# Openflight-sim/OPEN_Ludwig

Hardware: AMD Instinct MI355X
Metric: MLUPS (million lattice updates/s) at 256^3 D3Q27; % of HBM roofline (higher is better)
Workload: dtype f32

## Files before the change

open_ludwig_amd/csrc/kernels.hpp:

```cpp
#pragma once

#include <hip/hip_runtime.h>
#include <stdint.h>
#include <type_traits>

#include "lattice.hpp"
#include "jl_math.h"

namespace lw {

struct SCParams {
    const float *f_in;
    float *f_out;
    float *f_post;
    const uint32_t *post_rows;
    const float *vel_in;
    float *vel_out;
    float *rho;
    const uint8_t *obstacle;
    const float *sponge;
    const float *wall_dist;
    const int32_t *meta;
    const int32_t *items;
    const float *pf_new, *pf_old, *prho_new, *prho_old, *pvel_new, *pvel_old;
// ... 495 lines not shown

    const float tr_gsq = gsq11 + gsq22 + gsq33;
    const float tr_term = tr_gsq / 3.0f;
    const float Sd11 = gsq11 - tr_term, Sd22 = gsq22 - tr_term, Sd33 = gsq33 - tr_term;
    const float Sd12 = 0.5f * (gsq12 + gsq21), Sd13 = 0.5f * (gsq13 + gsq31), Sd23 = 0.5f * (gsq23 + gsq32);
    const float S12 = 0.5f * (g12 + g21), S13 = 0.5f * (g13 + g31), S23 = 0.5f * (g23 + g32);
    const float OP1 = Sd11 * Sd11 + Sd22 * Sd22 + Sd33 * Sd33 + 2.0f * (Sd12 * Sd12 + Sd13 * Sd13 + Sd23 * Sd23);
    const float OP2 = g11 * g11 + g22 * g22 + g33 * g33 + 2.0f * (S12 * S12 + S13 * S13 + S23 * S23);

    float nu_eddy = 0.0f;
    if (OP1 > 1.0e-12f) {
        const float OP1_32 = OP1 * sqrtf(OP1);
        const float OP2_52 = OP2 * OP2 * sqrtf(jl_max(OP2, 1.0e-12f));
        const float denom = OP2_52 + OP1 * sqrtf(sqrtf(jl_max(OP1, 1.0e-12f)));
        if (denom > 1.0e-12f) nu_eddy = (p.c_wale * p.c_wale) * OP1_32 / denom;
    }
    nu_eddy = jl_max(nu_eddy, p.nu_bg);
    const float tau_turb = p.tau + nu_eddy * 3.0f;
    const float omega = 1.0f / jl_max(tau_turb, 0.500001f);

    Chain2<PACKED> P_x, P_y, P_z;
    static_for<0, Q>([&](auto kc) {
        constexpr int k = decltype(kc)::value, ko = OPP(k);
        constexpr int cx = CX(k), cy = CY(k), cz = CZ(k);
        float f_neq;
        if constexpr (PACKED && k < ko) {
            const float cu = cdot<k>(ux_eq, uy_eq, uz_eq);
            const f32x2 both = f32x2{fs[k], fs[ko]} - equilibrium_value<f32x2>(rho, WEIGHT(k), f32x2{cu, -cu}, usq_eq);
            f_neq = both.x;
            fs[ko] = both.y;
        } else if constexpr (PACKED && k > ko) {
            f_neq = fs[k];
        } else {
            f_neq = fs[k] - equilibrium_value<float>(rho, WEIGHT(k), cdot<k>(ux_eq, uy_eq, uz_eq), usq_eq);
        }
        if constexpr (cx * cy != 0) P_x.add_both(f_neq, cx * cy > 0 ? f_neq : -f_neq);
        else if constexpr (cx != 0) P_x.add_first(f_neq);
        if constexpr (cy * cz != 0) P_y.add_both(f_neq, cy * cz > 0 ? f_neq : -f_neq);
        else if constexpr (cy != 0) P_y.add_first(f_neq);
        if constexpr (cz * cx != 0) P_z.add_both(f_neq, cz * cx > 0 ? f_neq : -f_neq);
        else if constexpr (cz != 0) P_z.add_first(f_neq);
    });
    const float Pi_xx = P_x.first(), Pi_xy = P_x.second(), Pi_yy = P_y.first(), Pi_yz = P_y.second(), Pi_zz = P_z.first(), Pi_zx = P_z.second();

    const float one_m_omega = 1.0f - omega;
    const float one_m_half_omega = 1.0f - 0.5f * omega;
    if constexpr (REC_OUT) {
        store_record(p.rec_out, own, rho, ux_eq, uy_eq, uz_eq, Pi_xx, Pi_yy, Pi_zz, Pi_xy, Pi_yz, Pi_zx, one_m_omega);
        return;
    }
    static_for<0, Q>([&](auto kc) {
        constexpr int k = decltype(kc)::value;
        float f_coll = collide_value<k>(rho, ux_eq, uy_eq, uz_eq, Pi_xx, Pi_yy, Pi_zz, Pi_xy, Pi_yz, Pi_zx, one_m_omega);
        if constexpr (WALL) {
            constexpr float w_k = WEIGHT(k);
            constexpr float cx_f = (float)CX(k), cy_f = (float)CY(k), cz_f = (float)CZ(k);
            const float cu = cdot<k>(ux_eq, uy_eq, uz_eq);
            const float force_term = (w_k * 3.0f) * ((cx_f - ux + 3.0f * cu * cx_f) * Fx + (cy_f - uy + 3.0f * cu * cy_f) * Fy +
                                                     (cz_f - uz + 3.0f * cu * cz_f) * Fz);
            f_coll = f_coll + one_m_half_omega * force_term;
        }
        if constexpr (POST) { if (store_post) st_f32(p.f_post, own.b, F_BLOCK_BYTES, k * COMP_BYTES + own.cell4, f_coll); }
        st_f32(p.f_out, own.b, F_BLOCK_BYTES, k * COMP_BYTES + own.cell4, f_coll);
    });
}

__device__ __forceinline__ void finish_rho_only(const SCParams &p, const int flags, const Own own, const float (&fs)[Q])
{
    float rho = 0.0f;
    static_for<0, Q>([&](auto kc) { rho += fs[decltype(kc)::value]; });
    bool is_obs = false;
    if (flags & FLAG_HAS_OBSTACLE) is_obs = p.obstacle[(size_t)own.b * CELLS + (own.cell4 >> 2)] != 0;
    if (is_obs) { st_f32(p.rho, own.b, S_BLOCK_BYTES, own.cell4, 1.0f); return; }
    rho = jl_max(rho, 0.01f);
    if (flags & FLAG_HAS_SPONGE) {
        const float sp = ld_own(p.sponge, own.b, S_BLOCK_BYTES, own.cell4);
        if (sp > 0.0f) rho = rho * (1.0f - sp) + 1.0f * sp;
    }
    st_f32(p.rho, own.b, S_BLOCK_BYTES, own.cell4, rho);
}

__device__ __forceinline__ void patch_missing_sources(const SCParams &p, const int32_t *__restrict__ meta, const NeighbourIds &nbr,
                                                      const LanePos &l, const int z, const Own own, float (&fs)[Q])
{
    const int gx = (meta[NBR_BX] - 1) * BS + l.x + 1, gy = (meta[NBR_BY] - 1) * BS + l.y + 1, gz = (meta[NBR_BZ] - 1) * BS + z + 1;
    const float *iface_own = p.is_level_1 == 0 ? p.f_iface + (size_t)meta[NBR_GBI] * CELLS + (own.cell4 >> 2) : nullptr;
    static_for<0, Q>([&](auto kc) {
        constexpr int k = decltype(kc)::value;
        constexpr int cx = CX(k), cy = CY(k), cz = CZ(k);
        if constexpr (k != 13) {
            if (source_block<k>(nbr, l) < 0) {
                const int src_gx = gx - cx, src_gy = gy - cy, src_gz = gz - cz;
                const bool is_inlet = src_gx < 1, is_outlet = src_gx > p.nx_g;
                const bool is_y_min = src_gy < 1, is_y_max = src_gy > p.ny_g;
                const bool is_z_min = src_gz < 1, is_z_max = src_gz > p.nz_g;
                float val;
                if (is_inlet) {
                    const float noise = p.inlet_turbulence > 0.0f
                                            ? gradient_noise(gy, gz, p.seed, 1234) * p.inlet_turbulence * p.u_inlet
                                            : 0.0f;
                    const float u_inst = p.u_inlet + noise;
                    const float cu_in = (float)cx * u_inst;
                    val = WEIGHT(k) * (1.0f + 3.0f * cu_in + 4.5f * cu_in * cu_in - 1.5f * u_inst * u_inst);
                } else if (is_outlet) {
                    const float cu_out = (float)cx * p.u_inlet;
                    val = WEIGHT(k) * (1.0f + 3.0f * cu_out + 4.5f * cu_out * cu_out - 1.5f * p.u_inlet * p.u_inlet);
                } else if (is_y_min && p.is_symmetric == 1) {
                    val = ld_own(p.f_in, own.b, F_BLOCK_BYTES, MIRROR_Y(k) * COMP_BYTES + own.cell4);
                } else if (is_y_min || is_y_max) {
                    val = ld_own(p.f_in, own.b, F_BLOCK_BYTES, MIRROR_Y(k) * COMP_BYTES + own.cell4);
                } else if (is_z_min || is_z_max) {
                    val = ld_own(p.f_in, own.b, F_BLOCK_BYTES, MIRROR_Z(k) * COMP_BYTES + own.cell4);
                } else if (p.is_level_1 == 0) {
                    val = iface_own[(size_t)k * p.n_iface_blocks * CELLS];
                } else {
                    val = WEIGHT(k);
                }
                fs[k] = val;
            }
        }
    });
}

__device__ __forceinline__ float dpp_from_lower_lane(float v)
{
    return __int_as_float(__builtin_amdgcn_update_dpp(__float_as_int(v), __float_as_int(v), 0x111, 0xF, 0xF, false));
}
__device__ __forceinline__ float dpp_from_upper_lane(float v)
{
    return __int_as_float(__builtin_amdgcn_update_dpp(__float_as_int(v), __float_as_int(v), 0x101, 0xF, 0xF, false));
}
__host__ __device__ constexpr int XSLOT(int k) { return CX(k) == 1 ? k / 3 : 9 + k / 3; }

constexpr int ITEM_LINK_W = 1 << 30;
constexpr int ITEM_LINK_E = 1 << 29;
constexpr int ITEM_ID_MASK = (1 << 29) - 1;

#ifndef LW_MIN_WAVES
#define LW_MIN_WAVES 5
#endif
template <int NW, bool GENERAL, bool POST, bool WALL, bool RHO_ONLY, bool WIDE, bool REC_OUT>
__device__ __forceinline__ void stream_collide_xrun(const SCParams p)
{
    __shared__ float xch[NW][24][8];
    const int wave = __builtin_amdgcn_readfirstlane(threadIdx.x >> 6);
    const int raw = p.items[blockIdx.x * NW + wave];
    const bool active = raw >= 0;
    const int item = active ? (raw & ITEM_ID_MASK) : 0;
    const int b = item >> 3;
    const int z = item & 7;
    const int lane = threadIdx.x & 63;
    LanePos l;
    l.x = lane & 7; l.y = lane >> 3;
    l.x0 = l.x == 0; l.x7 = l.x == 7; l.y0 = l.y == 0; l.y7 = l.y == 7;
    const int32_t *__restrict__ meta = p.meta + (size_t)b * NBR_STRIDE;
    const int flags = meta[NBR_FLAGS];
    const NeighbourIds nbr = load_neighbour_ids(meta, z);
    const Own own{b, (uint32_t)((l.x + 8 * l.y + 64 * z) * 4)};
    const bool first = !active || (raw & ITEM_LINK_W) == 0, last = !active || (raw & ITEM_LINK_E) == 0;
    float fs[Q];
    float halo[Q];
    float uc[3], uT[3], uB[3], uy_edge[3], ux_edge_lo[3], ux_edge_hi[3];
    if (active) {
    static_for<0, Q>([&](auto kc) {
        constexpr int k = decltype(kc)::value;
        constexpr int cx = CX(k), cy = CY(k), g = 1 - CZ(k);
        const bool yo = cy == 1 ? l.y0 : (cy == -1 ? l.y7 : false);
        const int c00 = nbr.id[g][4], cY = nbr.id[g][4 - 3 * cy];
        int sel = cy != 0 ? (yo ? cY : c00) : c00;
        if constexpr (GENERAL) sel = sel >= 0 ? sel : b;
        const uint32_t rowz = (uint32_t)(k * COMP_BYTES) + (uint32_t)((8 * ((l.y - cy) & 7)) * 4) + (uint32_t)(nbr.zs[g] * 256);
        if constexpr (cy == 0) fs[k] = ld_f32<true>(p.f_in, sel, F_BLOCK_BYTES, rowz + (uint32_t)(l.x * 4));
        else fs[k] = ld_f32<WIDE>(p.f_in, sel, F_BLOCK_BYTES, rowz + (uint32_t)(l.x * 4));
        halo[k] = 0.0f;
        if constexpr (cx != 0) {
            if (cx == 1 ? first : last) {
                const int cX = nbr.id[g][4 - cx], cXY = nbr.id[g][4 - cx - 3 * cy];
                int selx = cy != 0 ? (yo ? cXY : cX) : cX;
                if constexpr (GENERAL) selx = selx >= 0 ? selx : b;
                if (cx == 1 ? l.x0 : l.x7)
                    halo[k] = ld_f32<(cy == 0) || WIDE>(p.f_in, selx, F_BLOCK_BYTES, rowz + (uint32_t)((cx == 1 ? 7 : 0) * 4));
            }
        }
    });
    if constexpr (!RHO_ONLY) {
        int bT = z == 7 ? nbr.id[2][4] : b, bB = z == 0 ? nbr.id[0][4] : b;
        const uint32_t xy = (uint32_t)((l.x + 8 * l.y) * 4);
        uint32_t inT = xy + (uint32_t)(((z + 1) & 7) * 256), inB = xy + (uint32_t)(((z - 1) & 7) * 256);
        int by_ = l.y0 ? nbr.id[1][4 - 3] : nbr.id[1][4 + 3];
        uint32_t inY = (uint32_t)((l.x + 8 * (l.y0 ? 7 : 0) + 64 * z) * 4);
        int bXlo = nbr.id[1][4 - 1], bXhi = nbr.id[1][4 + 1];
        uint32_t inXlo = (uint32_t)((7 + 8 * l.y + 64 * z) * 4), inXhi = (uint32_t)((0 + 8 * l.y + 64 * z) * 4);
        if constexpr (GENERAL) {
            if (bT < 0) { bT = b; inT = own.cell4; }
            if (bB < 0) { bB = b; inB = own.cell4; }
            if (by_ < 0) { by_ = b; inY = own.cell4; }
            if (bXlo < 0) { bXlo = b; inXlo = own.cell4; }
            if (bXhi < 0) { bXhi = b; inXhi = own.cell4; }
        }
#pragma unroll
        for (int c = 0; c < 3; ++c) {
            const uint32_t cb = (uint32_t)c * COMP_BYTES;
            uc[c] = ld_own(p.vel_in, b, V_BLOCK_BYTES, cb + own.cell4);
            uT[c] = ld_own(p.vel_in, bT, V_BLOCK_BYTES, cb + inT);
            uB[c] = ld_own(p.vel_in, bB, V_BLOCK_BYTES, cb + inB);
            uy_edge[c] = 0.0f; ux_edge_lo[c] = 0.0f; ux_edge_hi[c] = 0.0f;
            if (l.y0 || l.y7) uy_edge[c] = ld_f32<WIDE>(p.vel_in, by_, V_BLOCK_BYTES, cb + inY);
            if (first) { if (l.x0) ux_edge_lo[c] = ld_own(p.vel_in, bXlo, V_BLOCK_BYTES, cb + inXlo); }
            if (last) { if (l.x7) ux_edge_hi[c] = ld_own(p.vel_in, bXhi, V_BLOCK_BYTES, cb + inXhi); }
        }
    }

    static_for<0, Q>([&](auto kc) {
        constexpr int k = decltype(kc)::value;
        constexpr int cx = CX(k);
        if constexpr (cx == 1) { if (l.x7) xch[wave][XSLOT(k)][l.y] = fs[k]; }
        if constexpr (cx == -1) { if (l.x0) xch[wave][XSLOT(k)][l.y] = fs[k]; }
    });
    if constexpr (!RHO_ONLY) {
#pragma unroll
        for (int c = 0; c < 3; ++c) {
            if (l.x7) xch[wave][18 + c][l.y] = uc[c];
            if (l.x0) xch[wave][21 + c][l.y] = uc[c];
        }
    }
    }
    __syncthreads();
    if (!active) return;
    const int wlo = first ? 0 : wave - 1, whi = last ? NW - 1 : wave + 1;
    static_for<0, Q>([&](auto kc) {
        constexpr int k = decltype(kc)::value;
        constexpr int cx = CX(k);
        if constexpr (cx == 1) {
            const float inner = dpp_from_lower_lane(fs[k]);
            const float edge = first ? halo[k] : xch[wlo][XSLOT(k)][l.y];
            fs[k] = l.x0 ? edge : inner;
        }
        if constexpr (cx == -1) {
            const float inner = dpp_from_upper_lane(fs[k]);
            const float edge = last ? halo[k] : xch[whi][XSLOT(k)][l.y];
            fs[k] = l.x7 ? edge : inner;
        }
    });
    const bool needs_patch = GENERAL && (flags & FLAG_ALL_NEIGHBOURS) == 0;
    if constexpr (RHO_ONLY) {
        if constexpr (GENERAL) { if (needs_patch) patch_missing_sources(p, meta, nbr, l, z, own, fs); }
        finish_rho_only(p, flags, own, fs);
        return;
    }
    float uE[3], uW[3], uN[3], uS[3];
#pragma unroll
    for (int c = 0; c < 3; ++c) {
        const float e_edge = last ? ux_edge_hi[c] : xch[whi][21 + c][l.y];
        const float w_edge = first ? ux_edge_lo[c] : xch[wlo][18 + c][l.y];
        const float e_in = dpp_from_upper_lane(uc[c]), w_in = dpp_from_lower_lane(uc[c]);
        uE[c] = l.x7 ? e_edge : e_in;
        uW[c] = l.x0 ? w_edge : w_in;
        const float n_in = __shfl_down(uc[c], 8, 64), s_in = __shfl_up(uc[c], 8, 64);
        uN[c] = l.y7 ? uy_edge[c] : n_in;
        uS[c] = l.y0 ? uy_edge[c] : s_in;
    }
    if constexpr (GENERAL) { if (needs_patch) patch_missing_sources(p, meta, nbr, l, z, own, fs); }
    finish_cell<POST, WALL, REC_OUT>(p, flags, own, fs, uE[0], uE[1], uE[2], uW[0], uW[1], uW[2], uN[0], uN[1], uN[2], uS[0], uS[1], uS[2],
                                     uT[0], uT[1], uT[2], uB[0], uB[1], uB[2]);
}
template <int NW, bool GENERAL, bool POST, bool WALL, bool RHO_ONLY = false, bool WIDE = false>
__global__ __launch_bounds__(64 * NW) __attribute__((amdgpu_waves_per_eu((WIDE && GENERAL) ? LW_MIN_WAVES - 1 : LW_MIN_WAVES))) void k_stream_collide_xrun(const SCParams p)
{
    stream_collide_xrun<NW, GENERAL, POST, WALL, RHO_ONLY, WIDE, false>(p);
}
template <int NW, bool WIDE>
__global__ __launch_bounds__(64 * NW) __attribute__((amdgpu_waves_per_eu(LW_MIN_WAVES))) void k_records_from_populations(const SCParams p)
{
    stream_collide_xrun<NW, false, false, false, false, WIDE, true>(p);
}

#ifndef LW_REC_WAVES
#define LW_REC_WAVES 4
#endif
#ifndef LW_REC_AHEAD
#define LW_REC_AHEAD 3
#endif
template <int NW, bool WIDE>
__global__ __launch_bounds__(64 * NW) __attribute__((amdgpu_waves_per_eu(LW_REC_WAVES))) void k_step_records(const SCParams p)
{
    __shared__ float xch[NW][24][8];
    const int wave = __builtin_amdgcn_readfirstlane(threadIdx.x >> 6);
    const int raw = p.items[blockIdx.x * NW + wave];
    const bool active = raw >= 0;
    const int item = active ? (raw & ITEM_ID_MASK) : 0;
    const int b = item >> 3;
    const int z = item & 7;
    const int lane = threadIdx.x & 63;
    LanePos l;
    l.x = lane & 7; l.y = lane >> 3;
    l.x0 = l.x == 0; l.x7 = l.x == 7; l.y0 = l.y == 0; l.y7 = l.y == 7;
    const int32_t *__restrict__ meta = p.meta + (size_t)b * NBR_STRIDE;
    const NeighbourIds nbr = load_neighbour_ids(meta, z);
    const Own own{b, (uint32_t)((l.x + 8 * l.y + 64 * z) * 4)};
    const bool first = !active || (raw & ITEM_LINK_W) == 0, last = !active || (raw & ITEM_LINK_E) == 0;
    __shared__ float xedge[NW][2][12][8];
    float fs[Q];
    float uc[3], uT[3], uB[3], uN[3], uS[3];
    if (active) {
    auto face_rows = [&](auto sc) {
        constexpr int side = decltype(sc)::value;
        constexpr int jx = side == 0 ? 4 - 1 : 4 + 1;
        const int j = l.x;
        const int jz = (j >= 3 ? 1 : 0) + (j >= 6 ? 1 : 0);
        const int cy = j - 3 * jz - 1, cz = jz - 1, g = 2 - jz;
        auto by_g = [&](int v0, int v1, int v2) { return g == 0 ? v0 : (g == 1 ? v1 : v2); };
        const int bX = by_g(nbr.id[0][jx], nbr.id[1][jx], nbr.id[2][jx]);
        const int bXlo = by_g(nbr.id[0][jx - 3], nbr.id[1][jx - 3], nbr.id[2][jx - 3]);
        const int bXhi = by_g(nbr.id[0][jx + 3], nbr.id[1][jx + 3], nbr.id[2][jx + 3]);
        const int blk = (cy == 1 && l.y0) ? bXlo : ((cy == -1 && l.y7) ? bXhi : bX);
        const int zsrc = by_g(nbr.zs[0], nbr.zs[1], nbr.zs[2]);
        float r[R_COMP];
        load_record_at(r, p.rec_in, record_offset<WIDE>(blk, zsrc) + (uint32_t)(((side == 0 ? 7 : 0) + 8 * ((l.y - cy) & 7)) * 4));
        float(&mine)[12][8] = xedge[wave][side];
        mine[j][l.y] = record_face(DirLaneFace{cy, cz}, r, side == 0);
        if (j == 4) { mine[9][l.y] = r[R_UX]; mine[10][l.y] = r[R_UY]; mine[11][l.y] = r[R_UZ]; }
    };
    if (first) face_rows(std::integral_constant<int, 0>{});
    if (last) face_rows(std::integral_constant<int, 1>{});
    if ((first && l.x0) || (last && l.x7)) {
        constexpr int j = 8, cy = 1, g = 0;
        const int wX = nbr.id[g][4 - 1], wXY = nbr.id[g][4 - 1 - 3 * cy], eX = nbr.id[g][4 + 1], eXY = nbr.id[g][4 + 1 - 3 * cy];
        const auto oW = record_offset<WIDE>(wX, nbr.zs[g]), oWY = record_offset<WIDE>(wXY, nbr.zs[g]);
        const auto oE = record_offset<WIDE>(eX, nbr.zs[g]), oEY = record_offset<WIDE>(eXY, nbr.zs[g]);
        const auto off = l.x0 ? (l.y0 ? oWY : oW) : (l.y0 ? oEY : oE);
        float r[R_COMP];
        load_record_at(r, p.rec_in, off + (uint32_t)(((l.x0 ? 7 : 0) + 8 * ((l.y - cy) & 7)) * 4));
        xedge[wave][l.x0 ? 0 : 1][j][l.y] = record_face(DirConst<DIR(1, 1, 1)>{}, r, l.x0);
    }
    __builtin_amdgcn_sched_barrier(0);
    {
        float r[9][R_COMP];
        auto load_pulled = [&](auto jc) {
            constexpr int j = decltype(jc)::value;
            constexpr int cy = j % 3 - 1, g = 1 - (j / 3 - 1);
            const uint32_t lane4 = (uint32_t)((l.x + 8 * ((l.y - cy) & 7)) * 4);
            if constexpr (cy == 0) {
                load_record(r[j], record_plane(p.rec_in, nbr.id[g][4], nbr.zs[g]), lane4);
            } else {
                const bool yo = cy == 1 ? l.y0 : l.y7;
                const auto o0 = record_offset<WIDE>(nbr.id[g][4], nbr.zs[g]), oY = record_offset<WIDE>(nbr.id[g][4 - 3 * cy], nbr.zs[g]);
                load_record_at(r[j], p.rec_in, (yo ? oY : o0) + lane4);
            }
        };
        static_for<0, LW_REC_AHEAD>(load_pulled);
        static_for<0, 9>([&](auto jc) {
            constexpr int j = decltype(jc)::value;
            constexpr int cy = j % 3 - 1, cz = j / 3 - 1;
            if constexpr (j + LW_REC_AHEAD < 9) load_pulled(std::integral_constant<int, j + LW_REC_AHEAD>{});
            __builtin_amdgcn_sched_barrier(0);
            const float(&q)[R_COMP] = r[j];
            record_row<cy, cz>(fs, q);
            if constexpr (cy == 0 && cz == 0) { uc[0] = q[R_UX]; uc[1] = q[R_UY]; uc[2] = q[R_UZ]; }
            if constexpr (cy == 0 && cz == 1) { uB[0] = q[R_UX]; uB[1] = q[R_UY]; uB[2] = q[R_UZ]; }
            if constexpr (cy == 0 && cz == -1) { uT[0] = q[R_UX]; uT[1] = q[R_UY]; uT[2] = q[R_UZ]; }
            if constexpr (cy == 1 && cz == 0) { uS[0] = q[R_UX]; uS[1] = q[R_UY]; uS[2] = q[R_UZ]; }
            if constexpr (cy == -1 && cz == 0) { uN[0] = q[R_UX]; uN[1] = q[R_UY]; uN[2] = q[R_UZ]; }
            __builtin_amdgcn_sched_barrier(0);
        });
    }
    static_for<0, Q>([&](auto kc) {
        constexpr int k = decltype(kc)::value;
        constexpr int cx = CX(k);
        if constexpr (cx == 1) { if (l.x7) xch[wave][XSLOT(k)][l.y] = fs[k]; }
        if constexpr (cx == -1) { if (l.x0) xch[wave][XSLOT(k)][l.y] = fs[k]; }
    });
#pragma unroll
    for (int c = 0; c < 3; ++c) {
        if (l.x7) xch[wave][18 + c][l.y] = uc[c];
        if (l.x0) xch[wave][21 + c][l.y] = uc[c];
    }
    }
    __syncthreads();
    if (!active) return;
    const int wlo = first ? 0 : wave - 1, whi = last ? NW - 1 : wave + 1;
    static_for<0, Q>([&](auto kc) {
        constexpr int k = decltype(kc)::value;
        constexpr int cx = CX(k);
        if constexpr (cx == 1) {
            const float inner = dpp_from_lower_lane(fs[k]);
            const float edge = first ? xedge[wave][0][k / 3][l.y] : xch[wlo][XSLOT(k)][l.y];
            fs[k] = l.x0 ? edge : inner;
        }
        if constexpr (cx == -1) {
            const float inner = dpp_from_upper_lane(fs[k]);
            const float edge = last ? xedge[wave][1][k / 3][l.y] : xch[whi][XSLOT(k)][l.y];
            fs[k] = l.x7 ? edge : inner;
        }
    });
    float uE[3], uW[3];
#pragma unroll
    for (int c = 0; c < 3; ++c) {
        const float e_edge = last ? xedge[wave][1][9 + c][l.y] : xch[whi][21 + c][l.y];
        const float w_edge = first ? xedge[wave][0][9 + c][l.y] : xch[wlo][18 + c][l.y];
        const float e_in = dpp_from_upper_lane(uc[c]), w_in = dpp_from_lower_lane(uc[c]);
        uE[c] = l.x7 ? e_edge : e_in;
        uW[c] = l.x0 ? w_edge : w_in;
    }
    finish_cell<false, false, true, true>(p, 0, own, fs, uE[0], uE[1], uE[2], uW[0], uW[1], uW[2], uN[0], uN[1], uN[2], uS[0], uS[1], uS[2],
                                    uT[0], uT[1], uT[2], uB[0], uB[1], uB[2]);
}

__global__ __launch_bounds__(256) void k_materialise(const SCParams p, int64_t n_cells)
{
    const int64_t i = (int64_t)blockIdx.x * 256 + threadIdx.x;
    if (i >= n_cells) return;
    const int b = (int)(i >> 9);
    const uint32_t cell = (uint32_t)(i & 511);
    float r[R_COMP];
    load_record(r, record_plane(p.rec_in, b, (int)(cell >> 6)), (cell & 63u) * 4);
    const Own own{b, cell * 4};
    st_f32(p.vel_out, b, V_BLOCK_BYTES, own.cell4, r[R_UX]);
    st_f32(p.vel_out, b, V_BLOCK_BYTES, COMP_BYTES + own.cell4, r[R_UY]);
    st_f32(p.vel_out, b, V_BLOCK_BYTES, 2 * COMP_BYTES + own.cell4, r[R_UZ]);
    if (p.rho) st_f32(p.rho, b, S_BLOCK_BYTES, own.cell4, r[R_RHO]);
    static_for<0, Q>([&](auto kc) {
        constexpr int k = decltype(kc)::value;
        st_f32(p.f_out, b, F_BLOCK_BYTES, k * COMP_BYTES + own.cell4,
               collide_value<k>(r[R_RHO], r[R_UX], r[R_UY], r[R_UZ], r[R_PXX], r[R_PYY], r[R_PZZ], r[R_PXY], r[R_PYZ], r[R_PZX], r[R_OMO]));
    });
}

__device__ __forceinline__ float weight_rt(int k)
{
    const int cx = k % 3 - 1, cy = (k / 3) % 3 - 1, cz = k / 9 - 1;
    const int d2 = cx * cx + cy * cy + cz * cz;
    return d2 == 0 ? WEIGHT(13) : d2 == 1 ? WEIGHT(12) : d2 == 2 ? WEIGHT(9) : WEIGHT(0);
}

struct InterfaceArgs {
    const int4 *corners;
    const float4 *weights;
    float4 *mac, *mac2;
    const int4 *links;
    float *f_iface2;
    float tw2;
    int n_sources, n_links;
};

__device__ __forceinline__ float blend_in_time(bool blend, float v_old, float v_new, float tw)
{
    return blend ? v_old * (1.0f - tw) + v_new * tw : v_new;
}

template <bool TWO>
__global__ __launch_bounds__(256) void k_interface_sources(const SCParams p, const InterfaceArgs a)
{
    const int i = blockIdx.x * 256 + threadIdx.x;
    if (i >= a.n_sources) return;
    const int4 c0 = a.corners[2 * i], c1 = a.corners[2 * i + 1];
    const int cc[8] = {c0.x, c0.y, c0.z, c0.w, c1.x, c1.y, c1.z, c1.w};
    const float4 w = a.weights[i];
    const float tw = p.temporal_weight, tw2 = a.tw2;
    const bool blend = p.use_temporal == 1 && tw < 0.99f, blend2 = TWO && p.use_temporal == 1 && tw2 < 0.99f;
    float v1[4][8], v2[4][8];
#pragma unroll
    for (int n = 0; n < 8; ++n) {
        v1[0][n] = 1.0f; v1[1][n] = 0.0f; v1[2][n] = 0.0f; v1[3][n] = 0.0f;
        v2[0][n] = 1.0f; v2[1][n] = 0.0f; v2[2][n] = 0.0f; v2[3][n] = 0.0f;
        if (cc[n] >= 0) {
            const int c = cc[n];
            const size_t cv = (size_t)(c >> 9) * (3 * CELLS) + (c & 511);
            const float vn[4] = {p.prho_new[c], p.pvel_new[cv], p.pvel_new[cv + CELLS], p.pvel_new[cv + 2 * CELLS]};
            float vo[4] = {0.0f, 0.0f, 0.0f, 0.0f};
            if (blend || blend2) { vo[0] = p.prho_old[c]; vo[1] = p.pvel_old[cv]; vo[2] = p.pvel_old[cv + CELLS]; vo[3] = p.pvel_old[cv + 2 * CELLS]; }
#pragma unroll
            for (int q = 0; q < 4; ++q) {
                v1[q][n] = blend_in_time(blend, vo[q], vn[q], tw);
                if (TWO) v2[q][n] = blend_in_time(blend2, vo[q], vn[q], tw2);
            }
        }
    }
#pragma unroll
    for (int n = 1; n < 8; ++n)
        if (cc[n] < 0) {
#pragma unroll
            for (int q = 0; q < 4; ++q) { v1[q][n] = v1[q][0]; v2[q][n] = v2[q][0]; }
        }
#define LW_TL(v, q) trilin(v[q][0], v[q][1], v[q][2], v[q][3], v[q][4], v[q][5], v[q][6], v[q][7], w.x, w.y, w.z)
    a.mac[i] = make_float4(LW_TL(v1, 0), LW_TL(v1, 1), LW_TL(v1, 2), LW_TL(v1, 3));
    if (TWO) a.mac2[i] = make_float4(LW_TL(v2, 0), LW_TL(v2, 1), LW_TL(v2, 2), LW_TL(v2, 3));
#undef LW_TL
}

template <bool TWO>
__global__ __launch_bounds__(256) void k_interface_links(const SCParams p, const InterfaceArgs a)
{
    const int j = blockIdx.x * 256 + threadIdx.x;
    if (j >= a.n_links) return;
    const int4 l = a.links[j];
    const int cell = l.x & 511, k = l.y & 31, gbi = l.y >> 5, src = l.z;
    const int4 c0 = a.corners[2 * src], c1 = a.corners[2 * src + 1];
    const int cc[8] = {c0.x, c0.y, c0.z, c0.w, c1.x, c1.y, c1.z, c1.w};
    const float4 w = a.weights[src];
    const float tw = p.temporal_weight, tw2 = a.tw2;
    const bool blend = p.use_temporal == 1 && tw < 0.99f, blend2 = TWO && p.use_temporal == 1 && tw2 < 0.99f;
    const float w_k = weight_rt(k);
    float fc[8], fc2[8];
#pragma unroll
    for (int n = 0; n < 8; ++n) {
        fc[n] = w_k; fc2[n] = w_k;
        if (cc[n] >= 0) {
            const size_t cf = ((size_t)(cc[n] >> 9) * Q + k) * CELLS + (cc[n] & 511);
            const float fn = p.pf_new[cf];
            float fo = 0.0f;
            if (blend || blend2) fo = p.pf_old[cf];
            fc[n] = blend_in_time(blend, fo, fn, tw);
            if (TWO) fc2[n] = blend_in_time(blend2, fo, fn, tw2);
        }
    }
#pragma unroll
    for (int n = 1; n < 8; ++n)
        if (cc[n] < 0) { fc[n] = fc[0]; fc2[n] = fc2[0]; }
    const float cxf = (float)(k % 3 - 1), cyf = (float)((k / 3) % 3 - 1), czf = (float)(k / 9 - 1);
    const float tau_c = p.tau_parent - 0.5f, tau_f = p.tau - 0.5f;
    const float scale = tau_c > 1.0e-6f ? jl_clamp(tau_f / tau_c, 0.01f, 100.0f) : 1.0f;
    const size_t out = ((size_t)k * p.n_iface_blocks + gbi) * CELLS + cell;
    {
        const float4 m = a.mac[src];
        const float f_int = trilin(fc[0], fc[1], fc[2], fc[3], fc[4], fc[5], fc[6], fc[7], w.x, w.y, w.z);
        const float feq_int = calculate_equilibrium(m.x, m.y, m.z, m.w, w_k, cxf, cyf, czf);
        const float f_neq = f_int - feq_int;
        p.f_iface[out] = feq_int + f_neq * scale;
    }
    if (TWO) {
        const float4 m = a.mac2[src];
        const float f_int = trilin(fc2[0], fc2[1], fc2[2], fc2[3], fc2[4], fc2[5], fc2[6], fc2[7], w.x, w.y, w.z);
        const float feq_int = calculate_equilibrium(m.x, m.y, m.z, m.w, w_k, cxf, cyf, czf);
        const float f_neq = f_int - feq_int;
        a.f_iface2[out] = feq_int + f_neq * scale;
    }
}


struct BouzidiParams {
    float *f_out;
    const float *f_post;
    const _Float16 *q_map;
    const int32_t *cell_block;
    const int8_t *cell_x, *cell_y, *cell_z;
    const int32_t *meta;
    int32_t n_cells;
    float q_min;
    const int4 *links;
    int32_t n_links;
};

__global__ __launch_bounds__(256) void k_bouzidi(const BouzidiParams p)
{
    const int i = blockIdx.x * 256 + threadIdx.x;
    auto at = [](int blk, int kk, int c) { return ((size_t)blk * Q + kk) * CELLS + c; };
    if (p.links) {
        if (i >= p.n_links) return;
        const int4 l = p.links[i];
        const float q = __int_as_float(l.z);
        if (!(q > p.q_min && q <= 1.0f)) return;
        const int b = l.x >> 9, cell = l.x & 511, k = l.y, opp_k = 26 - k;
        const float f_k = p.f_post[at(b, k, cell)];
        if (q < 0.5f) {
            const float f_ff = l.w >= 0 ? p.f_post[at(l.w >> 9, k, l.w & 511)] : f_k;
            const float coeff1 = 2.0f * q;
            p.f_out[at(b, opp_k, cell)] = coeff1 * f_k + (1.0f - coeff1) * f_ff;
        } else {
            const float f_opp_post = p.f_post[at(b, opp_k, cell)];
            const float inv_2q = 1.0f / (2.0f * q);
            const float coeff2 = (2.0f * q - 1.0f) * inv_2q;
            p.f_out[at(b, opp_k, cell)] = inv_2q * f_k + coeff2 * f_opp_post;
        }
        return;
    }
    int b, x, y, z, k;
    {
        if (i >= p.n_cells * Q) return;
        const int c = i / Q;
        k = i - c * Q;
        b = p.cell_block[c];
        x = p.cell_x[c]; y = p.cell_y[c]; z = p.cell_z[c];
    }
    const int opp_k = 26 - k;
    const int cell = x + 8 * y + 64 * z;
    const float q = (float)p.q_map[at(b, k, cell)];
    if (q > p.q_min && q <= 1.0f) {
        const float f_k = p.f_post[at(b, k, cell)];
        if (q < 0.5f) {
            const int nx = x + (opp_k % 3 - 1), ny = y + ((opp_k / 3) % 3 - 1), nz = z + (opp_k / 9 - 1);
            float f_ff = f_k;
            if (nx >= 0 && nx < BS && ny >= 0 && ny < BS && nz >= 0 && nz < BS) {
                f_ff = p.f_post[at(b, k, nx + 8 * ny + 64 * nz)];
            } else {
                const int ox = nx < 0 ? -1 : (nx >= BS ? 1 : 0);
                const int oy = ny < 0 ? -1 : (ny >= BS ? 1 : 0);
                const int oz = nz < 0 ? -1 : (nz >= BS ? 1 : 0);
                const int nbb = p.meta[(int64_t)b * NBR_STRIDE + DIR(ox, oy, oz)];
                if (nbb >= 0) f_ff = p.f_post[at(nbb, k, (nx & 7) + 8 * (ny & 7) + 64 * (nz & 7))];
            }
            const float coeff1 = 2.0f * q;
            p.f_out[at(b, opp_k, cell)] = coeff1 * f_k + (1.0f - coeff1) * f_ff;
        } else {
            const float f_opp_post = p.f_post[at(b, opp_k, cell)];
            const float inv_2q = 1.0f / (2.0f * q);
            const float coeff2 = (2.0f * q - 1.0f) * inv_2q;
            p.f_out[at(b, opp_k, cell)] = inv_2q * f_k + coeff2 * f_opp_post;
        }
    }
}

__global__ void k_fill_weights(float *f, int64_t n_cells)
{
    const int64_t i = (int64_t)blockIdx.x * blockDim.x + threadIdx.x;
    if (i >= n_cells) return;
    float *q = f + (i >> 9) * (int64_t)(Q * CELLS) + (i & 511);
    static_for<0, Q>([&](auto kc) {
        constexpr int k = decltype(kc)::value;
        q[k * CELLS] = WEIGHT(k);
    });
}
__global__ void k_fill(float *a, int64_t n, float v)
{
    const int64_t i = (int64_t)blockIdx.x * blockDim.x + threadIdx.x;
    if (i < n) a[i] = v;
}

struct SurfaceParams {
    const float *rho, *vel;
    const uint8_t *obstacle;
    const int32_t *block_pointer;
    int32_t gdx, gdy, gdz, n_tri, radius;
    float dx, tau, off_x, off_y, off_z, pressure_scale, stress_scale;
    const float *centers, *normals;
    float *p, *tx, *ty, *tz;
};

__device__ __forceinline__ void wall_stress(float rho, float ux, float uy, float uz, float nx, float ny, float nz, float wd, float tau,
                                            float pressure_scale, float stress_scale, float &p, float &sx, float &sy, float &sz)
{
    const float wall_dist = fmaxf(wd, 0.5f);
    p = ((rho - 1.0f) / 3.0f) * pressure_scale;
    const float udn = ux * nx + uy * ny + uz * nz;
    const float utx = ux - udn * nx, uty = uy - udn * ny, utz = uz - udn * nz;
    const float umag = sqrtf(utx * utx + uty * uty + utz * utz);
    const float nu_lat = (tau - 0.5f) / 3.0f;
    sx = 0.0f; sy = 0.0f; sz = 0.0f;
    if (umag > 1.0e-10f && wall_dist > 0.01f) {
        const float tmag = (rho * nu_lat * umag / wall_dist) * stress_scale;
        sx = (utx / umag) * tmag; sy = (uty / umag) * tmag; sz = (utz / umag) * tmag;
    }
}

__global__ __launch_bounds__(128) void k_map_stresses(const SurfaceParams s)
{
    const int i = blockIdx.x * 128 + threadIdx.x;
    if (i >= s.n_tri) return;
    const float tx = s.centers[3 * i] + s.off_x, ty = s.centers[3 * i + 1] + s.off_y, tz = s.centers[3 * i + 2] + s.off_z;
    const float nx = s.normals[3 * i], ny = s.normals[3 * i + 1], nz = s.normals[3 * i + 2];
    const int g_x = (int)floorf(tx / s.dx) + 1, g_y = (int)floorf(ty / s.dx) + 1, g_z = (int)floorf(tz / s.dx) + 1;
    float best_d = 1.0e10f, best_rho = 1.0f, ux = 0.0f, uy = 0.0f, uz = 0.0f, best_wd = 0.5f;
    bool found = false;
    for (int radius = 0; radius <= s.radius; ++radius) {
        if (found && radius > 1) break;
        for (int dz = -radius; dz <= radius; ++dz)
            for (int dy = -radius; dy <= radius; ++dy)
                for (int dx = -radius; dx <= radius; ++dx) {
                    if (radius > 0 && !(abs(dx) == radius || abs(dy) == radius || abs(dz) == radius)) continue;
                    const int cgx = g_x + dx, cgy = g_y + dy, cgz = g_z + dz;
                    if (cgx < 1 || cgy < 1 || cgz < 1) continue;
                    const int bx = (cgx - 1) / BS + 1, by = (cgy - 1) / BS + 1, bz = (cgz - 1) / BS + 1;
                    if (bx > s.gdx || by > s.gdy || bz > s.gdz) continue;
                    const int32_t b = s.block_pointer[(size_t)(bx - 1) + (size_t)s.gdx * ((size_t)(by - 1) + (size_t)s.gdy * (bz - 1))];
                    if (b <= 0) continue;
                    const int64_t c = (int64_t)((cgx - 1) % BS) + 8 * ((cgy - 1) % BS) + 64 * ((cgz - 1) % BS) + 512 * (int64_t)(b - 1);
                    if (s.obstacle[c]) continue;
                    const float ccx = ((float)cgx - 0.5f) * s.dx, ccy = ((float)cgy - 0.5f) * s.dx, ccz = ((float)cgz - 0.5f) * s.dx;
                    const float ex = tx - ccx, ey = ty - ccy, ez = tz - ccz;
                    const float d2 = ex * ex + ey * ey + ez * ez;
                    if (d2 < best_d) {
                        best_d = d2;
                        best_rho = s.rho[c];
// ... 1637 lines not shown
```

Measured before the change: 26950.

## Defer outer-face record loads past the main pull and evaluate after block barrier

```diff
diff --git a/open_ludwig_amd/csrc/kernels.hpp b/open_ludwig_amd/csrc/kernels.hpp
--- a/open_ludwig_amd/csrc/kernels.hpp
+++ b/open_ludwig_amd/csrc/kernels.hpp
@@ -821,38 +821,58 @@
     __shared__ float xedge[NW][2][12][8];
     float fs[Q];
     float uc[3], uT[3], uB[3], uN[3], uS[3];
-    if (active) {
-    auto face_rows = [&](auto sc) {
+    auto face_dir = [&](int &cy, int &cz) {
+        const int j = l.x;
+        const int jz = (j >= 3 ? 1 : 0) + (j >= 6 ? 1 : 0);
+        cy = j - 3 * jz - 1;
+        cz = jz - 1;
+    };
+    float rf[2][R_COMP], r9[R_COMP];
+    auto face_load = [&](auto sc) {
         constexpr int side = decltype(sc)::value;
         constexpr int jx = side == 0 ? 4 - 1 : 4 + 1;
-        const int j = l.x;
-        const int jz = (j >= 3 ? 1 : 0) + (j >= 6 ? 1 : 0);
-        const int cy = j - 3 * jz - 1, cz = jz - 1, g = 2 - jz;
+        int cy, cz;
+        face_dir(cy, cz);
+        const int g = 1 - cz;
         auto by_g = [&](int v0, int v1, int v2) { return g == 0 ? v0 : (g == 1 ? v1 : v2); };
         const int bX = by_g(nbr.id[0][jx], nbr.id[1][jx], nbr.id[2][jx]);
         const int bXlo = by_g(nbr.id[0][jx - 3], nbr.id[1][jx - 3], nbr.id[2][jx - 3]);
         const int bXhi = by_g(nbr.id[0][jx + 3], nbr.id[1][jx + 3], nbr.id[2][jx + 3]);
         const int blk = (cy == 1 && l.y0) ? bXlo : ((cy == -1 && l.y7) ? bXhi : bX);
         const int zsrc = by_g(nbr.zs[0], nbr.zs[1], nbr.zs[2]);
-        float r[R_COMP];
-        load_record_at(r, p.rec_in, record_offset<WIDE>(blk, zsrc) + (uint32_t)(((side == 0 ? 7 : 0) + 8 * ((l.y - cy) & 7)) * 4));
+        load_record_at(rf[side], p.rec_in, record_offset<WIDE>(blk, zsrc) + (uint32_t)(((side == 0 ? 7 : 0) + 8 * ((l.y - cy) & 7)) * 4));
+    };
+    auto face_eval = [&](auto sc) {
+        constexpr int side = decltype(sc)::value;
+        int cy, cz;
+        face_dir(cy, cz);
+        const int j = l.x;
+        const float(&r)[R_COMP] = rf[side];
         float(&mine)[12][8] = xedge[wave][side];
         mine[j][l.y] = record_face(DirLaneFace{cy, cz}, r, side == 0);
         if (j == 4) { mine[9][l.y] = r[R_UX]; mine[10][l.y] = r[R_UY]; mine[11][l.y] = r[R_UZ]; }
     };
-    if (first) face_rows(std::integral_constant<int, 0>{});
-    if (last) face_rows(std::integral_constant<int, 1>{});
-    if ((first && l.x0) || (last && l.x7)) {
-        constexpr int j = 8, cy = 1, g = 0;
+    const bool ninth = (first && l.x0) || (last && l.x7);
+    auto ninth_load = [&]() {
+        constexpr int cy = 1, g = 0;
         const int wX = nbr.id[g][4 - 1], wXY = nbr.id[g][4 - 1 - 3 * cy], eX = nbr.id[g][4 + 1], eXY = nbr.id[g][4 + 1 - 3 * cy];
         const auto oW = record_offset<WIDE>(wX, nbr.zs[g]), oWY = record_offset<WIDE>(wXY, nbr.zs[g]);
         const auto oE = record_offset<WIDE>(eX, nbr.zs[g]), oEY = record_offset<WIDE>(eXY, nbr.zs[g]);
         const auto off = l.x0 ? (l.y0 ? oWY : oW) : (l.y0 ? oEY : oE);
-        float r[R_COMP];
-        load_record_at(r, p.rec_in, off + (uint32_t)(((l.x0 ? 7 : 0) + 8 * ((l.y - cy) & 7)) * 4));
-        xedge[wave][l.x0 ? 0 : 1][j][l.y] = record_face(DirConst<DIR(1, 1, 1)>{}, r, l.x0);
-    }
-    __builtin_amdgcn_sched_barrier(0);
+        load_record_at(r9, p.rec_in, off + (uint32_t)(((l.x0 ? 7 : 0) + 8 * ((l.y - cy) & 7)) * 4));
+    };
+    auto ninth_eval = [&]() { xedge[wave][l.x0 ? 0 : 1][8][l.y] = record_face(DirConst<DIR(1, 1, 1)>{}, r9, l.x0); };
+    auto outer_face_loads = [&]() {
+        if (first) face_load(std::integral_constant<int, 0>{});
+        if (last) face_load(std::integral_constant<int, 1>{});
+        if (ninth) ninth_load();
+    };
+    auto outer_face_evals = [&]() {
+        if (first) face_eval(std::integral_constant<int, 0>{});
+        if (last) face_eval(std::integral_constant<int, 1>{});
+        if (ninth) ninth_eval();
+    };
+    if (active) {
     {
         float r[9][R_COMP];
         auto load_pulled = [&](auto jc) {
@@ -894,9 +914,14 @@
         if (l.x7) xch[wave][18 + c][l.y] = uc[c];
         if (l.x0) xch[wave][21 + c][l.y] = uc[c];
     }
+    outer_face_loads();
     }
     __syncthreads();
     if (!active) return;
+    outer_face_evals();
+    __builtin_amdgcn_fence(__ATOMIC_RELEASE, "wavefront");
+    __builtin_amdgcn_wave_barrier();
+    __builtin_amdgcn_fence(__ATOMIC_ACQUIRE, "wavefront");
     const int wlo = first ? 0 : wave - 1, whi = last ? NW - 1 : wave + 1;
     static_for<0, Q>([&](auto kc) {
         constexpr int k = decltype(kc)::value;
```

Result: faster. 27700, median of 6 (+2.8%).
